# ydixon/yolo_v3

Measured on AMD Instinct MI355X. Metric: images/sec (YOLOv3 forward + decode + NMS, 416x416, bs=64 per GPU), higher is better.
Workload: dtype f32 (exact fp32 MFMA); 1 GPU; 416x416 bs=64 per GPU, 64 distinct synthetic scenes per GPU, SW-1 synthetic weights, conf=0.50 nms=0.40; global_batch=64, parallelism=dp1, entry=Detector.run_device, lanes=2

## Files before the change

### yolo_v3_amd/csrc/conv_wino4_f32.hip

```cpp
#include <type_traits>
#include "yv3_common.h"

namespace {

#define W4F_GPTR(p) ((const __attribute__((address_space(1))) void*)(p))
#define W4F_LPTR(p) ((__attribute__((address_space(3))) void*)(p))

typedef float f32x2 __attribute__((ext_vector_type(2)));

constexpr int BNC = 64;
constexpr int BMT = 32;
constexpr int ROWB = 128;
constexpr int U_BYTES = BNC * ROWB;
constexpr int V_BYTES = BMT * ROWB;
constexpr int STAGE = U_BYTES + V_BYTES;
#define W4F_NSTAGE 4
#ifndef W4F_PRIO
#define W4F_PRIO 3
#endif
#ifndef W4F_EXTRA_LDS
#define W4F_EXTRA_LDS 0
#endif
#ifndef W4F_DMA_FIRST
#define W4F_DMA_FIRST 0
#endif
constexpr int NSTAGE = W4F_NSTAGE;
#if defined(YV3_MEASURE) && defined(W4F_ABL)
constexpr int ABL = W4F_ABL;
#else
constexpr int ABL = 0;
#endif

struct Wino4Params {
    const float* v;
    const float* u;
    const float* alpha;
    const float* beta;
    const float* res;
    float* y;
    int C, Cout, H, W, th, tw, T;
    int cchunks;
    int nblk_n;
    int act;
    long long pos_stride;
    unsigned u_bytes, v_bytes;
    int nitems, n_full, parts;
    float* sk_parts;
    int* sk_flags;
    int* status;
};
constexpr int W4F_MAX_TAIL_WG = 2 * YV3_WINO_SK_MAX_WG - 1;
constexpr int W4F_PART_FLOATS = 4 * 32 * 256;

template <int N> __device__ __forceinline__ void w4f_wait_vmcnt() { asm volatile("s_waitcnt vmcnt(%0)" :: "n"(N) : "memory"); }

__device__ __forceinline__ int w4f_swz(int row) { return (row >> 1) & 7; }

__device__ __forceinline__ void bt_apply(const f32x4 (&d)[6], f32x4 (&o)[6]) {
    o[0] = d[0] - 1.5f * d[1] - 2.0f * d[2] + 1.5f * d[3] + d[4];
    o[1] = 0.5f * d[2] - d[1] + 2.5f * d[3] + d[4];
    o[2] = d[1] - 2.5f * d[2] + 0.5f * d[3] + d[4];
    o[3] = 2.0f * (d[3] - d[1]) - d[2] + d[4];
    o[4] = 0.5f * (d[1] - d[3]) - d[2] + d[4];
    o[5] = d[1] - 1.5f * d[2] - 2.0f * d[3] + 1.5f * d[4] + d[5];
}

__global__ __launch_bounds__(256) void wino4_input_f32_kernel(const float* __restrict__ x, float* __restrict__ v,
                                                              int H, int W, int C, int th, int tw, long long T) {
    const int cg = C >> 2;
    const long long i = (long long)blockIdx.x * blockDim.x + threadIdx.x;
    if (i >= T * cg) return;
    const long long t = i / cg;
    const int c = (int)(i - t * cg) * 4;
    const int b = (int)(t / (th * tw));
    const int rem = (int)(t - (long long)b * th * tw);
    const int ty = rem / tw, tx = rem - ty * tw;
    const int y0 = 4 * ty - 1, x0 = 4 * tx - 1;
    f32x4 tr[6][6];
#pragma unroll
    for (int r = 0; r < 6; ++r) {
        f32x4 d[6];
        const int yy = y0 + r;
#pragma unroll
        for (int q = 0; q < 6; ++q) {
            const int xx = x0 + q;
            const bool ok = (unsigned)yy < (unsigned)H && (unsigned)xx < (unsigned)W;
            d[q] = ok ? *reinterpret_cast<const f32x4*>(x + (((long long)b * H + yy) * W + xx) * C + c) : f32x4{0.f, 0.f, 0.f, 0.f};
        }
        bt_apply(d, tr[r]);
    }
#pragma unroll
    for (int l = 0; l < 6; ++l) {
        f32x4 col[6], o[6];
#pragma unroll
        for (int r = 0; r < 6; ++r) col[r] = tr[r][l];
        bt_apply(col, o);
#pragma unroll
        for (int xi = 0; xi < 6; ++xi) *reinterpret_cast<f32x4*>(v + ((long long)(xi * 6 + l) * T + t) * C + c) = o[xi];
    }
}

__global__ __launch_bounds__(256) void wino4_pack_kernel(const float* __restrict__ u, float* __restrict__ out, int cout, int cin) {
    const long long i = (long long)blockIdx.x * blockDim.x + threadIdx.x;
    const long long n4 = (long long)cout * cin * 36 / 4;
    if (i >= n4) return;
    const int cch = cin / 32;
    const int ps = (int)(i & 7);
    const int row = (int)((i >> 3) & 63);
    long long r = i >> 9;
    const int cc = (int)(r % cch); r /= cch;
    const int pos = (int)(r % 36);
    const int nb = (int)(r / 36);
    const int slot = ps ^ w4f_swz(row);
    const int o = nb * 64 + row, c = cc * 32 + slot * 4;
    f32x4 q;
#pragma unroll
    for (int e = 0; e < 4; ++e) q[e] = u[((long long)o * cin + c + e) * 36 + pos];
    *reinterpret_cast<f32x4*>(out + i * 4) = q;
}

__device__ __forceinline__ constexpr float at_coef(int j, int nu) {
    return nu == 0 ? (j == 0 ? 1.f : 0.f)
         : nu == 1 ? 1.f
         : nu == 2 ? ((j & 1) ? -1.f : 1.f)
         : nu == 3 ? (j == 0 ? 1.f : j == 1 ? 0.5f : j == 2 ? 0.25f : 0.125f)
         : nu == 4 ? (j == 0 ? 1.f : j == 1 ? -2.f : j == 2 ? 4.f : -8.f)
         : (j == 3 ? 1.f : 0.f);
}

template <bool CCH2, bool SK>
__global__ __launch_bounds__(256, 2) void conv_wino4_f32_kernel(const Wino4Params p) {
    extern __shared__ __attribute__((aligned(16))) unsigned char lds[];
    const int tid = threadIdx.x;
    const int lane = tid & 63;
    const int wid = __builtin_amdgcn_readfirstlane(tid >> 6);
    const int nk = 36 * p.cchunks;
    const int nkx = 6 * p.cchunks;
#if defined(YV3_MEASURE) && defined(W4F_DEPHASE)
    if (blockIdx.x >= 256 && blockIdx.x < 512)
        for (int i = 0; i < nk * W4F_DEPHASE / 5000; ++i) __builtin_amdgcn_s_sleep(108);
#endif

    int item, xa = 0, xb = 6, sk_t = 0;
    if (!SK || (int)blockIdx.x < p.n_full) item = yv3_xcd_remap(blockIdx.x, SK ? p.n_full : (int)gridDim.x);
    else {
        sk_t = blockIdx.x - p.n_full;
        const int nt = p.nitems - p.n_full;
        const int x = sk_t & 7, l = sk_t >> 3;
        const int i0 = (int)(((long long)nt * x) >> 3), i1 = (int)(((long long)nt * (x + 1)) >> 3);
        const int il = l / p.parts, part = l - il * p.parts;
        if (il >= i1 - i0) return;
        item = p.n_full + i0 + il;
        const int rows = 6 / p.parts;
        xa = part * rows; xb = xa + rows;
    }

    const __amdgpu_buffer_rsrc_t urs = __builtin_amdgcn_make_buffer_rsrc(const_cast<float*>(p.u), 0, (int)p.u_bytes, 0x00020000);
    const __amdgpu_buffer_rsrc_t vrs = __builtin_amdgcn_make_buffer_rsrc(const_cast<float*>(p.v), 0, (int)p.v_bytes, 0x00020000);
    unsigned usoff = 0;
    const unsigned uoff = lane * 16;
    unsigned vsoff = 0, voff = 0;
    int pf_c = 0;
    int pf_k = 0, pf_end = 0;
    auto dma_piece = [&](int i, unsigned char* stage) {
        if (ABL & 8) return;
        if (i == 0)      __builtin_amdgcn_raw_ptr_buffer_load_lds(urs, W4F_LPTR(stage + (2 * wid) * 1024), 16, uoff, usoff, 0, 0);
        else if (i == 1) __builtin_amdgcn_raw_ptr_buffer_load_lds(urs, W4F_LPTR(stage + (2 * wid) * 1024), 16, uoff, usoff, 1024, 0);
        else             __builtin_amdgcn_raw_ptr_buffer_load_lds(vrs, W4F_LPTR(stage + U_BYTES + wid * 1024), 16, voff, vsoff, 0, 0);
    };
    auto dma_advance = [&]() {
        if (pf_k + 1 < pf_end) {
            ++pf_k;
            usoff += BNC * 32 * 4;
            vsoff += 128;
            pf_c += 32;
            if (pf_c == p.C) { pf_c = 0; vsoff += (unsigned)(p.pos_stride - p.C) * 4u; }
        }
    };

    const int fr = lane & 15, fq = lane >> 4;
    const int urow = 16 * wid + fr;
    const int u_off0 = urow * ROWB + ((fq ^ w4f_swz(urow)) << 4);
    const int u_off1 = urow * ROWB + (((4 + fq) ^ w4f_swz(urow)) << 4);
    int v_off0[2], v_off1[2];
#pragma unroll
    for (int b = 0; b < 2; ++b) {
        const int r = 16 * b + fr;
        v_off0[b] = U_BYTES + r * ROWB + ((fq ^ w4f_swz(r)) << 4);
        v_off1[b] = U_BYTES + r * ROWB + (((4 + fq) ^ w4f_swz(r)) << 4);
    }

    f32x4 P[2], R[4][2], Y[4][4][2];
    struct Frag { f32x4 ua, va0, va1, ub, vb0, vb1; };
    auto read_frag = [&](const unsigned char* st) {
        Frag f;
        if (ABL & 4) { f.ua = f.va0 = f.va1 = f.ub = f.vb0 = f.vb1 = f32x4{(float)lane, 1.f, 2.f, 3.f}; return f; }
        f.ua = *reinterpret_cast<const f32x4*>(st + u_off0);
        f.va0 = *reinterpret_cast<const f32x4*>(st + v_off0[0]);
        f.va1 = *reinterpret_cast<const f32x4*>(st + v_off0[1]);
        f.ub = *reinterpret_cast<const f32x4*>(st + u_off1);
        f.vb0 = *reinterpret_cast<const f32x4*>(st + v_off1[0]);
        f.vb1 = *reinterpret_cast<const f32x4*>(st + v_off1[1]);
        return f;
    };
    Frag F0, F1;
    using TrueT = std::integral_constant<bool, true>;
    using FalseT = std::integral_constant<bool, false>;

#if defined(YV3_MEASURE) && defined(W4F_TIMELINE)
    unsigned long long tl_t = __builtin_amdgcn_s_memtime(), tl_sync = 0, tl_burst = 0, tl_fold = 0;
    const unsigned long long tl_entry = tl_t;
#define W4F_MARK(acc_) do { const unsigned long long t_ = __builtin_amdgcn_s_memtime(); acc_ += t_ - tl_t; tl_t = t_; } while (0)
#else
#define W4F_MARK(acc_) do {} while (0)
#endif
    auto chunk = [&](auto first_c, auto stage_c, const Frag& F, Frag& G) {
        constexpr bool FIRST = decltype(first_c)::value;
        constexpr int S = decltype(stage_c)::value;
        const f32x4 zero4 = {0.f, 0.f, 0.f, 0.f};
        W4F_MARK(tl_fold);
        w4f_wait_vmcnt<3 * (NSTAGE - 2)>();
        __builtin_amdgcn_s_waitcnt(0xC07F);
        if (!(ABL & 16)) __builtin_amdgcn_s_barrier();
        __builtin_amdgcn_sched_barrier(0);
        W4F_MARK(tl_sync);
        unsigned char* const fr_ = lds + S * STAGE;
        G = read_frag(lds + ((S + 1) % NSTAGE) * STAGE);
#if W4F_PRIO == 3
        __builtin_amdgcn_s_setprio(1);
#endif
#pragma unroll
        for (int t = 0; t < 4; ++t) {
            if (ABL & 2) { P[0][t] += F.ua[t] + F.va0[t]; P[1][t] += F.va1[t]; }
            else {
            P[0] = __builtin_amdgcn_mfma_f32_16x16x4f32(F.ua[t], F.va0[t], (FIRST && t == 0) ? zero4 : P[0], 0, 0, 0);
            P[1] = __builtin_amdgcn_mfma_f32_16x16x4f32(F.ua[t], F.va1[t], (FIRST && t == 0) ? zero4 : P[1], 0, 0, 0);
            }
            __builtin_amdgcn_sched_barrier(0);
            if (t < 3) dma_piece(t, fr_);
            __builtin_amdgcn_sched_barrier(0);
        }
#pragma unroll
        for (int t = 0; t < 4; ++t) {
            if (ABL & 2) { P[0][t] += F.ub[t] + F.vb0[t]; P[1][t] += F.vb1[t]; }
            else {
            P[0] = __builtin_amdgcn_mfma_f32_16x16x4f32(F.ub[t], F.vb0[t], P[0], 0, 0, 0);
            P[1] = __builtin_amdgcn_mfma_f32_16x16x4f32(F.ub[t], F.vb1[t], P[1], 0, 0, 0);
            }
        }
#if W4F_PRIO == 3
        __builtin_amdgcn_s_setprio(0);
#endif
        dma_advance();
        W4F_MARK(tl_burst);
    };

    auto position = [&](auto nu_c) {
        constexpr int nu = decltype(nu_c)::value;
        {
            using S0 = std::integral_constant<int, 0>; using S1 = std::integral_constant<int, 1>;
            using S2 = std::integral_constant<int, 2>; using S3 = std::integral_constant<int, 3>;
            if constexpr (CCH2) {
                if constexpr ((nu & 1) == 0) { chunk(TrueT{}, S0{}, F0, F1); chunk(FalseT{}, S1{}, F1, F0); }
                else                         { chunk(TrueT{}, S2{}, F0, F1); chunk(FalseT{}, S3{}, F1, F0); }
            } else {
                chunk(TrueT{}, S0{}, F0, F1); chunk(FalseT{}, S1{}, F1, F0); chunk(FalseT{}, S2{}, F0, F1); chunk(FalseT{}, S3{}, F1, F0);
                for (int cc = 4; cc < p.cchunks; cc += 4) {
                    chunk(FalseT{}, S0{}, F0, F1); chunk(FalseT{}, S1{}, F1, F0); chunk(FalseT{}, S2{}, F0, F1); chunk(FalseT{}, S3{}, F1, F0);
                }
            }
            if (ABL & 32) return;
#pragma unroll
            for (int b = 0; b < 2; ++b) {
#pragma unroll
                for (int j = 0; j < 4; ++j) {
                    constexpr float z = 0.f;
                    const float cf = at_coef(j, nu);
                    if (cf != z) {
#pragma unroll
                        for (int e = 0; e < 4; ++e) R[j][b][e] = fmaf(P[b][e], cf, R[j][b][e]);
                    }
                }
            }
        }
    };
    {
        const int nb = item % p.nblk_n;
        const int n0 = nb * BNC;
        const int m0 = (item / p.nblk_n) * BMT;
        {
            const int k0 = xa * nkx;
            usoff = (unsigned)((((long long)nb * nk + k0) * (BNC * 32) + (2 * wid) * 256) * 4);
            const int vrow = 8 * wid + (lane >> 3);
            const int vt = min(m0 + vrow, p.T - 1);
            vsoff = (unsigned)m0 * (unsigned)p.C * 4u + (unsigned)(6 * xa) * (unsigned)p.pos_stride * 4u;
            voff = (unsigned)(vt - m0) * (unsigned)p.C * 4u + ((((unsigned)lane & 7u) ^ (unsigned)w4f_swz(vrow)) << 4);
            pf_c = 0; pf_k = k0; pf_end = xb * nkx;
        }
#pragma unroll
        for (int b = 0; b < 2; ++b) {
            P[b] = f32x4{0.f, 0.f, 0.f, 0.f};
#pragma unroll
            for (int j = 0; j < 4; ++j) {
                R[j][b] = f32x4{0.f, 0.f, 0.f, 0.f};
#pragma unroll
                for (int i = 0; i < 4; ++i) Y[i][j][b] = f32x4{0.f, 0.f, 0.f, 0.f};
            }
        }
#pragma unroll
        for (int d = 0; d < NSTAGE; ++d) {
#pragma unroll
            for (int i = 0; i < 3; ++i) dma_piece(i, lds + d * STAGE);
            dma_advance();
        }
        w4f_wait_vmcnt<3 * (NSTAGE - 1)>();
        __builtin_amdgcn_s_barrier();
#if W4F_PRIO == 1
        if (__builtin_amdgcn_s_getreg((3 << 11) | 4) & 1) __builtin_amdgcn_s_setprio(2);
#elif W4F_PRIO == 2
        if ((blockIdx.x >> 8) & 1) __builtin_amdgcn_s_setprio(2);
#endif
        F0 = read_frag(lds);
        for (int xi = xa; xi < xb; ++xi) {
            position(std::integral_constant<int, 0>{}); position(std::integral_constant<int, 1>{}); position(std::integral_constant<int, 2>{});
            position(std::integral_constant<int, 3>{}); position(std::integral_constant<int, 4>{}); position(std::integral_constant<int, 5>{});
            const float c1 = xi == 0 || xi == 5 ? 0.f : xi == 1 ? 1.f : xi == 2 ? -1.f : xi == 3 ? 0.5f : -2.f;
            const float cfi[4] = {xi == 5 ? 0.f : 1.f, c1, c1 * c1, xi == 5 ? 1.f : c1 * c1 * c1};
#pragma unroll
            for (int i = 0; i < 4; ++i) {
                if (cfi[i] == 0.f) continue;
#pragma unroll
                for (int j = 0; j < 4; ++j)
#pragma unroll
                    for (int b = 0; b < 2; ++b)
#pragma unroll
                        for (int e = 0; e < 4; ++e) Y[i][j][b][e] = fmaf(R[j][b][e], cfi[i], Y[i][j][b][e]);
            }
#pragma unroll
            for (int j = 0; j < 4; ++j)
#pragma unroll
                for (int b = 0; b < 2; ++b) R[j][b] = f32x4{0.f, 0.f, 0.f, 0.f};
        }
        w4f_wait_vmcnt<0>();
#if defined(YV3_MEASURE) && defined(W4F_TIMELINE)
        const unsigned long long tl_loop_end = __builtin_amdgcn_s_memtime();
#endif

        if constexpr (SK) {
            if (xa == 0 && xb < 6) {
                for (int k = 1; k < p.parts; ++k) {
                    const int partner = sk_t + 8 * k;
                    if (tid == 0) {
                        int n = 0, f;
                        while ((f = __hip_atomic_load(p.sk_flags + partner, __ATOMIC_RELAXED, __HIP_MEMORY_SCOPE_AGENT)) == 0 && ++n < (1 << 22))
                            __builtin_amdgcn_s_sleep(2);
                        if ((f == 0 || f != 1 + (int)(__builtin_amdgcn_s_getreg((3 << 11) | 20) & 15)) && p.status) atomicOr(p.status, 2);
                        __hip_atomic_store(p.sk_flags + partner, 0, __ATOMIC_RELAXED, __HIP_MEMORY_SCOPE_AGENT);
                    }
                    __syncthreads();
                    const float* w = p.sk_parts + (size_t)partner * W4F_PART_FLOATS + wid * (32 * 256) + lane * 4;
#pragma unroll
                    for (int i = 0; i < 4; ++i) {
                        f32x4 t[4][2];
#pragma unroll
                        for (int j = 0; j < 4; ++j)
#pragma unroll
                            for (int b = 0; b < 2; ++b) t[j][b] = *reinterpret_cast<const f32x4*>(w + ((i * 4 + j) * 2 + b) * 256);
#pragma unroll
                        for (int j = 0; j < 4; ++j)
#pragma unroll
                            for (int b = 0; b < 2; ++b) Y[i][j][b] += t[j][b];
                        __builtin_amdgcn_sched_barrier(0);
                    }
                }
            }
        }

        const bool raw = SK && xa > 0;
        const int cw = n0 + 16 * wid + 4 * fq;
        const f32x4 one4 = {1.f, 1.f, 1.f, 1.f}, zero4 = {0.f, 0.f, 0.f, 0.f};
        const f32x4 al = raw ? one4 : *reinterpret_cast<const f32x4*>(p.alpha + cw);
        const f32x4 be = raw ? zero4 : *reinterpret_cast<const f32x4*>(p.beta + cw);
        const bool leaky = !raw && p.act == YV3_ACT_LEAKY;
        const float* const res = raw ? nullptr : p.res;
        float* const ybase = raw ? p.sk_parts + (size_t)sk_t * W4F_PART_FLOATS + wid * (32 * 256) + lane * 4 : p.y;
        long long pix[2];
        int py[2], px[2];
#pragma unroll
        for (int b = 0; b < 2; ++b) {
            const int t = m0 + 16 * b + fr;
            if (t < p.T) {
                const int tt = p.th * p.tw;
                const int bi = t / tt, rem = t - bi * tt;
                const int ty = rem / p.tw, tx = rem - ty * p.tw;
                py[b] = 4 * ty; px[b] = 4 * tx;
                pix[b] = ((long long)bi * p.H + py[b]) * p.W + px[b];
            } else { pix[b] = -1; py[b] = px[b] = 0; }
        }
        auto out_off = [&](int i, int j, int b) -> long long {
            if (raw) return ((i * 4 + j) * 2 + b) * 256;
            const bool ok = pix[b] >= 0 && py[b] + i < p.H && px[b] + j < p.W;
            return ok ? (pix[b] + (long long)i * p.W + j) * p.Cout + cw : -1;
        };
        f32x4 rr[2][4][2];
        auto load_res = [&](int i) {
#pragma unroll
            for (int j = 0; j < 4; ++j)
#pragma unroll
                for (int b = 0; b < 2; ++b) {
                    const long long off = out_off(i, j, b);
                    rr[i & 1][j][b] = off >= 0 ? *reinterpret_cast<const f32x4*>(res + off) : f32x4{0.f, 0.f, 0.f, 0.f};
                }
        };
        if (res) load_res(0);
#pragma unroll
        for (int i = 0; i < ((ABL & 1) ? 1 : 4); ++i) {
            if (res && i + 1 < 4) load_res(i + 1);
#pragma unroll
            for (int j = 0; j < 4; ++j)
#pragma unroll
                for (int b = 0; b < 2; ++b) {
                    const long long off = out_off(i, j, b);
                    f32x4 q;
#pragma unroll
                    for (int e = 0; e < 4; ++e) {
                        float v = fmaf(Y[i][j][b][e], al[e], be[e]);
                        if (leaky) v = v > 0.f ? v : 0.1f * v;
                        q[e] = res ? v + rr[i & 1][j][b][e] : v;
                    }
                    if (off >= 0) *reinterpret_cast<f32x4*>(ybase + off) = q;
                }
        }
        if (raw) {
            asm volatile("s_waitcnt vmcnt(0)" ::: "memory");
            __syncthreads();
            if (tid == 0) __hip_atomic_store(p.sk_flags + sk_t, 1 + (int)(__builtin_amdgcn_s_getreg((3 << 11) | 20) & 15),
                                             __ATOMIC_RELAXED, __HIP_MEMORY_SCOPE_AGENT);
        }
#if defined(YV3_MEASURE) && defined(W4F_TIMELINE)
        if (blockIdx.x == W4F_TIMELINE && lane == 0) {
            const unsigned long long tl_end = __builtin_amdgcn_s_memtime();
            __builtin_amdgcn_s_waitcnt(0);
            float* dbg = p.y + wid * 8;
            dbg[0] = (float)tl_sync / nk; dbg[1] = (float)tl_burst / nk; dbg[2] = (float)tl_fold / nk; dbg[3] = (float)(tl_loop_end - tl_entry);
            dbg[4] = (float)(tl_end - tl_loop_end); dbg[5] = (float)nk;
        }
#endif
    }
}

}

extern "C" int yv3_pack_wino4_weight_f32(const float* u_oc66, float* packed, int cout, int cin, void* stream) {
    if (!u_oc66 || !packed || cout <= 0 || cin <= 0) return YV3_EINVAL;
    if (cout % 64 || (cin != 64 && cin % 128)) return YV3_ESHAPE;
    const long long n4 = (long long)cout * cin * 9;
    hipLaunchKernelGGL(wino4_pack_kernel, dim3((unsigned)((n4 + 255) / 256)), dim3(256), 0, (hipStream_t)stream, u_oc66, packed, cout, cin);
    YV3_CHECK_LAUNCH();
    return 0;
}

static size_t wino4_v_bytes(int B, int H, int W, int cin) { return (size_t)36 * B * ((H + 3) / 4) * ((W + 3) / 4) * cin * sizeof(float); }
extern "C" size_t yv3_wino4_workspace_bytes(int B, int H, int W, int cin) {
    if (B <= 0 || H <= 0 || W <= 0 || cin <= 0) return 0;
    return ((wino4_v_bytes(B, H, W, cin) + 255) & ~(size_t)255) + yv3_wino_sk_bytes();
}

long long yv3_wino4_f32_workgroups(const yv3_conv_desc* d) {
    const long long T = (long long)d->B * ((d->H + 3) / 4) * ((d->W + 3) / 4);
    return ((T + BMT - 1) / BMT) * (d->cout / BNC);
}

static long long wino4_tail_cost(long long tail, int P, int nkx, int ncu, bool lone_only) {
    const long long W = tail * P;
    if (P > 1 && (8 * ((tail + 7) / 8) * P > W4F_MAX_TAIL_WG || (lone_only && W > ncu))) return -1;
    const long long f = W <= ncu ? 1 : W <= 2 * ncu ? 2 : 2 * ((W + 2 * ncu - 1) / (2 * ncu));
    return (6 / P) * nkx * f + (P > 1 ? 29 + 5 * P : 0);
}
static void wino4_schedule(const yv3_conv_desc* d, long long items, int* n_full, int* parts) {
    const int ncu = yv3_num_cu(), slots = 2 * ncu;
    *n_full = (int)items; *parts = 1;
    if ((d->options & YV3_OPT_WINO4_TILES) || d->tune[1] == 1 || items < 1) return;
    const long long full = d->tune[1] == 2 ? 0 : (items / slots) * slots;
    const long long tail = items - full;
    if (tail == 0) return;
    const int nkx = 6 * (d->cin / 32);
    int best = 1; long long best_cost = wino4_tail_cost(tail, 1, nkx, ncu, false);
    for (int P = 2; P <= 6; ++P) {
        if (6 % P) continue;
        const long long c = wino4_tail_cost(tail, P, nkx, ncu, full > 0);
        if (c >= 0 && c < best_cost) { best = P; best_cost = c; }
    }
    if ((d->tune[2] == 2 || d->tune[2] == 3 || d->tune[2] == 6) && wino4_tail_cost(tail, d->tune[2], nkx, ncu, false) >= 0) best = d->tune[2];
    if (best == 1) return;
    *n_full = (int)full; *parts = best;
}

bool yv3_wino4_f32_pays(const yv3_conv_desc* d) {
    const long long items = yv3_wino4_f32_workgroups(d), ncu = yv3_num_cu();
    if ((d->options & YV3_OPT_WINO4_TILES) || d->tune[1] == 1) return items * 10 >= 3 * ncu;
    return d->cin >= 256 ? true : d->cin == 128 ? items * 100 >= 17 * ncu : items * 100 >= 39 * ncu;
}

int yv3_conv2d_wino4_f32(const yv3_conv_desc* d, hipStream_t s) {
    const int th = (d->H + 3) / 4, tw = (d->W + 3) / 4;
    const long long T = (long long)d->B * th * tw;
    if (T > 0x7fffffffLL || d->cout % BNC || d->cout_pad != d->cout || (d->cin != 64 && d->cin % 128) || d->k != 3 || d->stride != 1 || d->cin_up) return YV3_ESHAPE;
    if (!d->w_wino4) return YV3_EINVAL;
    if (!d->wino_ws || d->wino_ws_bytes < yv3_wino4_workspace_bytes(d->B, d->H, d->W, d->cin)) return YV3_EWORKSPACE;
    float* v = (float*)d->wino_ws;
    {
        const long long n = T * (d->cin >> 2);
        hipLaunchKernelGGL(wino4_input_f32_kernel, dim3((unsigned)((n + 255) / 256)), dim3(256), 0, s, (const float*)d->x, v, d->H, d->W, d->cin, th, tw, T);
        YV3_CHECK_LAUNCH();
    }
    Wino4Params p;
    p.v = v; p.u = (const float*)d->w_wino4;
    p.alpha = d->alpha; p.beta = d->beta; p.res = (const float*)d->residual; p.y = (float*)d->y;
    p.C = d->cin; p.Cout = d->cout; p.H = d->H; p.W = d->W; p.th = th; p.tw = tw; p.T = (int)T;
    p.cchunks = d->cin / 32; p.nblk_n = d->cout / BNC; p.act = d->act;
    p.pos_stride = T * d->cin;
    if (!p.alpha) return YV3_EINVAL;
    const unsigned long long vb = 36ull * T * d->cin * 4, ub = 36ull * d->cout * d->cin * 4;
    if (vb > 0xffffffffull || ub > 0xffffffffull) return YV3_ESHAPE;
    p.u_bytes = (unsigned)ub; p.v_bytes = (unsigned)vb;
    const long long items = ((T + BMT - 1) / BMT) * p.nblk_n;
    if (items * 6 > 0x7fffffffLL) return YV3_ESHAPE;
    p.nitems = (int)items;
    wino4_schedule(d, items, &p.n_full, &p.parts);
    char* area = (char*)d->wino_ws + ((d->wino_ws_bytes - yv3_wino_sk_bytes()) & ~(size_t)255);
    p.sk_parts = (float*)area;
    p.sk_flags = (int*)(area + (size_t)W4F_MAX_TAIL_WG * W4F_PART_FLOATS * sizeof(float));
    p.status = d->flags;
    const size_t lds = (size_t)NSTAGE * STAGE + W4F_EXTRA_LDS;
    if (p.parts > 1) {
        const long long tail = items - p.n_full;
        const dim3 grid((unsigned)(p.n_full + 8 * ((tail + 7) / 8) * p.parts));
        if (p.cchunks == 2) hipLaunchKernelGGL((conv_wino4_f32_kernel<true, true>), grid, dim3(256), lds, s, p);
        else                hipLaunchKernelGGL((conv_wino4_f32_kernel<false, true>), grid, dim3(256), lds, s, p);
    } else {
        const dim3 grid((unsigned)items);
        if (p.cchunks == 2) hipLaunchKernelGGL((conv_wino4_f32_kernel<true, false>), grid, dim3(256), lds, s, p);
        else                hipLaunchKernelGGL((conv_wino4_f32_kernel<false, false>), grid, dim3(256), lds, s, p);
    }
    YV3_CHECK_LAUNCH();
    return 0;
}
```

Baseline: 3268 images/sec.

## Load Winograd filter fragments directly into registers via a ring instead of LDS

Filter (U) tiles are no longer DMA'd into LDS. Each wave now loads its own MFMA A-fragments straight from global memory into a ring of registers, several chunks ahead. The pack kernel reorders the filter layout so each lane's 16-byte load matches its MFMA fragment, and LDS stages shrink to only the input (V) tile. This cuts LDS traffic, LDS footprint and the LDS reads for U, which may allow more occupancy. The cost is extra VGPRs for the ring and vmcnt bookkeeping that must stay correct across mixed register and LDS loads.

```diff
diff --git a/yolo_v3_amd/csrc/conv_wino4_f32.hip b/yolo_v3_amd/csrc/conv_wino4_f32.hip
--- a/yolo_v3_amd/csrc/conv_wino4_f32.hip
+++ b/yolo_v3_amd/csrc/conv_wino4_f32.hip
@@ -13,7 +13,7 @@
 constexpr int ROWB = 128;
 constexpr int U_BYTES = BNC * ROWB;
 constexpr int V_BYTES = BMT * ROWB;
-constexpr int STAGE = U_BYTES + V_BYTES;
+constexpr int STAGE = V_BYTES;
 #define W4F_NSTAGE 4
 #ifndef W4F_PRIO
 #define W4F_PRIO 3
@@ -25,6 +25,12 @@
 #define W4F_DMA_FIRST 0
 #endif
 constexpr int NSTAGE = W4F_NSTAGE;
+#ifndef W4F_URING
+#define W4F_URING 4
+#endif
+constexpr int URING = W4F_URING;
+constexpr int ULEAD = URING - 1;
+static_assert(URING == 2 || URING == 4, "the filter ring follows the stage index");
 #if defined(YV3_MEASURE) && defined(W4F_ABL)
 constexpr int ABL = W4F_ABL;
 #else
@@ -105,14 +111,13 @@
     const long long n4 = (long long)cout * cin * 36 / 4;
     if (i >= n4) return;
     const int cch = cin / 32;
-    const int ps = (int)(i & 7);
-    const int row = (int)((i >> 3) & 63);
+    const int l = (int)(i & 63);
+    const int h = (int)((i >> 6) & 1), w = (int)((i >> 7) & 3);
     long long r = i >> 9;
     const int cc = (int)(r % cch); r /= cch;
     const int pos = (int)(r % 36);
     const int nb = (int)(r / 36);
-    const int slot = ps ^ w4f_swz(row);
-    const int o = nb * 64 + row, c = cc * 32 + slot * 4;
+    const int o = nb * 64 + 16 * w + (l & 15), c = cc * 32 + 16 * h + 4 * (l >> 4);
     f32x4 q;
 #pragma unroll
     for (int e = 0; e < 4; ++e) q[e] = u[((long long)o * cin + c + e) * 36 + pos];
@@ -162,16 +167,23 @@
     unsigned vsoff = 0, voff = 0;
     int pf_c = 0;
     int pf_k = 0, pf_end = 0;
-    auto dma_piece = [&](int i, unsigned char* stage) {
+    int pu_k = 0;
+    f32x4 UA[URING], UB[URING];
+    auto u_load = [&](int h, int s) {
         if (ABL & 8) return;
-        if (i == 0)      __builtin_amdgcn_raw_ptr_buffer_load_lds(urs, W4F_LPTR(stage + (2 * wid) * 1024), 16, uoff, usoff, 0, 0);
-        else if (i == 1) __builtin_amdgcn_raw_ptr_buffer_load_lds(urs, W4F_LPTR(stage + (2 * wid) * 1024), 16, uoff, usoff, 1024, 0);
-        else             __builtin_amdgcn_raw_ptr_buffer_load_lds(vrs, W4F_LPTR(stage + U_BYTES + wid * 1024), 16, voff, vsoff, 0, 0);
-    };
-    auto dma_advance = [&]() {
+        const auto q = __builtin_amdgcn_raw_buffer_load_b128(urs, h ? uoff + 1024 : uoff, usoff, 0);
+        (h ? UB[s] : UA[s]) = __builtin_bit_cast(f32x4, q);
+    };
+    auto v_piece = [&](unsigned char* stage) {
+        if (ABL & 8) return;
+        __builtin_amdgcn_raw_ptr_buffer_load_lds(vrs, W4F_LPTR(stage + wid * 1024), 16, voff, vsoff, 0, 0);
+    };
+    auto u_advance = [&]() {
+        if (pu_k + 1 < pf_end) { ++pu_k; usoff += U_BYTES; }
+    };
+    auto v_advance = [&]() {
         if (pf_k + 1 < pf_end) {
             ++pf_k;
-            usoff += BNC * 32 * 4;
             vsoff += 128;
             pf_c += 32;
             if (pf_c == p.C) { pf_c = 0; vsoff += (unsigned)(p.pos_stride - p.C) * 4u; }
@@ -179,26 +191,21 @@
     };
 
     const int fr = lane & 15, fq = lane >> 4;
-    const int urow = 16 * wid + fr;
-    const int u_off0 = urow * ROWB + ((fq ^ w4f_swz(urow)) << 4);
-    const int u_off1 = urow * ROWB + (((4 + fq) ^ w4f_swz(urow)) << 4);
     int v_off0[2], v_off1[2];
 #pragma unroll
     for (int b = 0; b < 2; ++b) {
         const int r = 16 * b + fr;
-        v_off0[b] = U_BYTES + r * ROWB + ((fq ^ w4f_swz(r)) << 4);
-        v_off1[b] = U_BYTES + r * ROWB + (((4 + fq) ^ w4f_swz(r)) << 4);
+        v_off0[b] = r * ROWB + ((fq ^ w4f_swz(r)) << 4);
+        v_off1[b] = r * ROWB + (((4 + fq) ^ w4f_swz(r)) << 4);
     }
 
     f32x4 P[2], R[4][2], Y[4][4][2];
-    struct Frag { f32x4 ua, va0, va1, ub, vb0, vb1; };
+    struct Frag { f32x4 va0, va1, vb0, vb1; };
     auto read_frag = [&](const unsigned char* st) {
         Frag f;
-        if (ABL & 4) { f.ua = f.va0 = f.va1 = f.ub = f.vb0 = f.vb1 = f32x4{(float)lane, 1.f, 2.f, 3.f}; return f; }
-        f.ua = *reinterpret_cast<const f32x4*>(st + u_off0);
+        if (ABL & 4) { f.va0 = f.va1 = f.vb0 = f.vb1 = f32x4{(float)lane, 1.f, 2.f, 3.f}; return f; }
         f.va0 = *reinterpret_cast<const f32x4*>(st + v_off0[0]);
         f.va1 = *reinterpret_cast<const f32x4*>(st + v_off0[1]);
-        f.ub = *reinterpret_cast<const f32x4*>(st + u_off1);
         f.vb0 = *reinterpret_cast<const f32x4*>(st + v_off1[0]);
         f.vb1 = *reinterpret_cast<const f32x4*>(st + v_off1[1]);
         return f;
@@ -207,6 +214,7 @@
     using TrueT = std::integral_constant<bool, true>;
     using FalseT = std::integral_constant<bool, false>;
 
+    constexpr int VMCNT_LOOP = ULEAD == NSTAGE - 1 ? 3 * (NSTAGE - 2) : 1;
 #if defined(YV3_MEASURE) && defined(W4F_TIMELINE)
     unsigned long long tl_t = __builtin_amdgcn_s_memtime(), tl_sync = 0, tl_burst = 0, tl_fold = 0;
     const unsigned long long tl_entry = tl_t;
@@ -219,39 +227,41 @@
         constexpr int S = decltype(stage_c)::value;
         const f32x4 zero4 = {0.f, 0.f, 0.f, 0.f};
         W4F_MARK(tl_fold);
-        w4f_wait_vmcnt<3 * (NSTAGE - 2)>();
+        w4f_wait_vmcnt<VMCNT_LOOP>();
         __builtin_amdgcn_s_waitcnt(0xC07F);
         if (!(ABL & 16)) __builtin_amdgcn_s_barrier();
         __builtin_amdgcn_sched_barrier(0);
         W4F_MARK(tl_sync);
         unsigned char* const fr_ = lds + S * STAGE;
         G = read_frag(lds + ((S + 1) % NSTAGE) * STAGE);
+        const f32x4 ua = UA[S % URING], ub = UB[S % URING];
 #if W4F_PRIO == 3
         __builtin_amdgcn_s_setprio(1);
 #endif
 #pragma unroll
         for (int t = 0; t < 4; ++t) {
-            if (ABL & 2) { P[0][t] += F.ua[t] + F.va0[t]; P[1][t] += F.va1[t]; }
+            if (ABL & 2) { P[0][t] += ua[t] + F.va0[t]; P[1][t] += F.va1[t]; }
             else {
-            P[0] = __builtin_amdgcn_mfma_f32_16x16x4f32(F.ua[t], F.va0[t], (FIRST && t == 0) ? zero4 : P[0], 0, 0, 0);
-            P[1] = __builtin_amdgcn_mfma_f32_16x16x4f32(F.ua[t], F.va1[t], (FIRST && t == 0) ? zero4 : P[1], 0, 0, 0);
+            P[0] = __builtin_amdgcn_mfma_f32_16x16x4f32(ua[t], F.va0[t], (FIRST && t == 0) ? zero4 : P[0], 0, 0, 0);
+            P[1] = __builtin_amdgcn_mfma_f32_16x16x4f32(ua[t], F.va1[t], (FIRST && t == 0) ? zero4 : P[1], 0, 0, 0);
             }
             __builtin_amdgcn_sched_barrier(0);
-            if (t < 3) dma_piece(t, fr_);
+            if (t < 2) u_load(t, (S + ULEAD) % URING);
+            else if (t == 2) v_piece(fr_);
             __builtin_amdgcn_sched_barrier(0);
         }
 #pragma unroll
         for (int t = 0; t < 4; ++t) {
-            if (ABL & 2) { P[0][t] += F.ub[t] + F.vb0[t]; P[1][t] += F.vb1[t]; }
+            if (ABL & 2) { P[0][t] += ub[t] + F.vb0[t]; P[1][t] += F.vb1[t]; }
             else {
-            P[0] = __builtin_amdgcn_mfma_f32_16x16x4f32(F.ub[t], F.vb0[t], P[0], 0, 0, 0);
-            P[1] = __builtin_amdgcn_mfma_f32_16x16x4f32(F.ub[t], F.vb1[t], P[1], 0, 0, 0);
+            P[0] = __builtin_amdgcn_mfma_f32_16x16x4f32(ub[t], F.vb0[t], P[0], 0, 0, 0);
+            P[1] = __builtin_amdgcn_mfma_f32_16x16x4f32(ub[t], F.vb1[t], P[1], 0, 0, 0);
             }
         }
 #if W4F_PRIO == 3
         __builtin_amdgcn_s_setprio(0);
 #endif
-        dma_advance();
+        u_advance(); v_advance();
         W4F_MARK(tl_burst);
     };
 
@@ -295,7 +305,7 @@
             const int vt = min(m0 + vrow, p.T - 1);
             vsoff = (unsigned)m0 * (unsigned)p.C * 4u + (unsigned)(6 * xa) * (unsigned)p.pos_stride * 4u;
             voff = (unsigned)(vt - m0) * (unsigned)p.C * 4u + ((((unsigned)lane & 7u) ^ (unsigned)w4f_swz(vrow)) << 4);
-            pf_c = 0; pf_k = k0; pf_end = xb * nkx;
+            pf_c = 0; pf_k = pu_k = k0; pf_end = xb * nkx;
         }
 #pragma unroll
         for (int b = 0; b < 2; ++b) {
@@ -307,13 +317,17 @@
                 for (int i = 0; i < 4; ++i) Y[i][j][b] = f32x4{0.f, 0.f, 0.f, 0.f};
             }
         }
-#pragma unroll
-        for (int d = 0; d < NSTAGE; ++d) {
-#pragma unroll
-            for (int i = 0; i < 3; ++i) dma_piece(i, lds + d * STAGE);
-            dma_advance();
-        }
-        w4f_wait_vmcnt<3 * (NSTAGE - 1)>();
+        if (ABL & 8) {
+#pragma unroll
+            for (int s = 0; s < URING; ++s) UA[s] = UB[s] = f32x4{(float)lane, 1.f, 2.f, 3.f};
+        }
+#pragma unroll
+        for (int j = -NSTAGE; j < 0; ++j) {
+            if (j + ULEAD >= 0) { u_load(0, (j + ULEAD) % URING); u_load(1, (j + ULEAD) % URING); u_advance(); }
+            v_piece(lds + (j + NSTAGE) * STAGE);
+            v_advance();
+        }
+        w4f_wait_vmcnt<3 * (NSTAGE - 1) + 2 * (ULEAD - NSTAGE + 1)>();
         __builtin_amdgcn_s_barrier();
 #if W4F_PRIO == 1
         if (__builtin_amdgcn_s_getreg((3 << 11) | 4) & 1) __builtin_amdgcn_s_setprio(2);
```

New measurement: 3269 images/sec (median of 2 runs). Within noise of the previous version (+0.0%).
